# ownzonefeng/pytorch-distributed-training-example

Hardware: AMD Instinct MI355X
Metric: images/sec (whole node) ResNet-50 DDP at 1/2/4/8 MI355X; scaling efficiency (higher is better)
Workload: dtype bf16; 1 GPU; model=resnet50, global_batch=1024, per_gpu_batch=1024, image_size=224, parallelism=dp1, grad_accum=1, impl=ours, graph=False, precision=bf16, bucket_cap_mb=auto, comm_hook=none, reducer_active=True, pg_size=1, pg_backend=nccl, deterministic=False, full=False

## Files before the change

### pytorch_distributed_training_example_amd/config.py

```python
from __future__ import annotations

import os


class _Switches:
    __slots__ = ("disable_native", "conv1x1", "conv1x1_ours", "conv1x1_prefer", "conv1x1_override",
                 "conv1x1_table", "conv1x1_dump", "conv1x1_s2", "conv3x3", "conv3x3_wgrad", "conv3x3_s2", "conv_stem",
                 "conv_bn_stats", "bn_bwd_stats", "res_masked", "stem_bwd_fused", "stem_bn_wgrad", "stem_bn_stats", "stem_pool_wgrad", "wgrad_splitk", "slice_sum",
                 "subsample_native", "linear_splitk", "fused_addln", "embedding_native", "linear_epilogue",
                 "bwd_fused", "bwd_fused_shapes", "bwd_alg", "alg_glo", "bwd_alg_min_m", "z3_virtual", "bwd_alg_first", "ds_alg", "bn2_defer", "bn_apply_gemm_k", "strided_bstats", "gap_native", "sub_out",
                 "fp8_fused_gelu", "fp8_weight_multi", "fp8_cast_colsum", "fp8_ln", "wgrad_stream_m",
                 "dropout_fused")

    def __init__(self):
        self.reload()

    def reload(self) -> "_Switches":
        e = os.environ.get

        def on(name: str, default: str = "1") -> bool:
            return e(name, default) != "0"

        self.disable_native = e("PDT_DISABLE_NATIVE", "0") == "1"
        self.conv1x1 = e("PDT_CONV1X1", "auto")
# ... 2 lines not shown
        ov = e("PDT_CONV1X1_OVERRIDE", "")
        self.conv1x1_override = dict(p.split("=", 1) for p in ov.replace("+", ";").split(";") if "=" in p)
        self.conv1x1_table = on("PDT_CONV1X1_TABLE")
        self.conv1x1_dump = e("PDT_CONV1X1_DUMP") or None
        self.conv1x1_s2 = e("PDT_CONV1X1_S2", "1") == "1"
        self.conv3x3 = e("PDT_CONV3X3", "ours")
        self.conv3x3_wgrad = e("PDT_CONV3X3_WGRAD", "ours")
        self.conv3x3_s2 = e("PDT_CONV3X3_S2", "ours")
        self.conv_stem = e("PDT_CONV_STEM", "ours")
        self.conv_bn_stats = on("PDT_CONV_BN_STATS")
        self.bn_bwd_stats = on("PDT_BN_BWD_STATS")
        self.res_masked = on("PDT_RES_MASKED")
        self.stem_bwd_fused = on("PDT_STEM_BWD_FUSED")
        self.stem_bn_wgrad = on("PDT_STEM_BN_WGRAD")
        self.stem_bn_stats = on("PDT_STEM_BN_STATS")
        self.stem_pool_wgrad = on("PDT_STEM_POOL_WGRAD")
        self.wgrad_splitk = on("PDT_WGRAD_SPLITK")
        self.slice_sum = on("PDT_SLICE_SUM")
        self.subsample_native = on("PDT_SUBSAMPLE_NATIVE")
        self.linear_splitk = on("PDT_LINEAR_SPLITK")
        self.fused_addln = on("PDT_FUSED_ADDLN")
        self.embedding_native = on("PDT_EMBEDDING_NATIVE")
        self.linear_epilogue = e("PDT_LINEAR_EPILOGUE", "auto")
        self.bwd_fused = on("PDT_BWD_FUSED")
        self.bwd_fused_shapes = tuple(tuple(int(v) for v in t.split("x")) for t in
                                      e("PDT_BWD_FUSED_SHAPES", "256x64").split(",") if "x" in t)
        self.bwd_alg = int(e("PDT_BWD_ALG", "2"))
        self.bwd_alg_min_m = int(e("PDT_BWD_ALG_MIN_M", "50176"))
        self.alg_glo = on("PDT_ALG_GLO", "1")
        self.z3_virtual = int(e("PDT_Z3_VIRTUAL", "2"))
        self.bwd_alg_first = on("PDT_BWD_ALG_FIRST", "1")
        self.ds_alg = int(e("PDT_DS_ALG", "512"))
        self.bn2_defer = on("PDT_BN2_DEFER", "0")
        self.bn_apply_gemm_k = int(e("PDT_BN_APPLY_GEMM_K", "128"))
        self.strided_bstats = on("PDT_STRIDED_BSTATS")
        self.gap_native = on("PDT_GAP_NATIVE")
        self.sub_out = on("PDT_SUB_OUT")
        self.fp8_fused_gelu = on("PDT_FP8_FUSED_GELU")
        self.fp8_weight_multi = on("PDT_FP8_WEIGHT_MULTI")
        self.fp8_cast_colsum = on("PDT_FP8_CAST_COLSUM")
        self.fp8_ln = on("PDT_FP8_LN")
        self.wgrad_stream_m = int(e("PDT_WGRAD_STREAM_M", "0"))
        self.dropout_fused = on("PDT_DROPOUT_FUSED")
        return self


SW = _Switches()
```

### pytorch_distributed_training_example_amd/csrc/binding.cpp

```cpp
#include <torch/extension.h>
#include <ATen/hip/HIPContext.h>

#include <cstring>
#include <map>
#include <vector>

#include "fp8_pack.h"
#include "launchers.h"

namespace {

using at::Tensor;

hipStream_t stream() { return at::hip::getCurrentHIPStream().stream(); }

int dcode(const Tensor& t) {
  if (t.scalar_type() == at::kFloat) return 0;
  if (t.scalar_type() == at::kBFloat16) return 1;
  TORCH_CHECK(false, "pdt: unsupported dtype ", t.scalar_type(), " (fp32 / bf16 only)");
}

void check_cuda(const Tensor& t, const char* name) {
  TORCH_CHECK(t.is_cuda(), "pdt: ", name, " must be a GPU tensor");
}
// ... 2306 lines not shown
  m.doc() = "gfx950 HIP kernels for pytorch_distributed_training_example_amd";
  m.def("sgd", &sgd);
  m.def("adam", &adam);
  m.def("adadelta", &adadelta);
  m.def("lars", &lars);
  m.def("lamb", &lamb);
  m.def("layerwise_chunks", &layerwise_chunks);
  m.def("amp_unscale", &amp_unscale);
  m.def("amp_update", &amp_update);
  m.def("mt_scale", &mt_scale);
  m.def("mt_copy", &mt_copy);
  m.def("l2norm_sq", &l2norm_sq);
  m.def("clip_coef", &clip_coef);
  m.def("bn_tune", [](int variant, int target_blocks, int u_fwd, int u_bwd) {
    if (pdt_bn_tune(variant, target_blocks, u_fwd, u_bwd) != 0)
      throw py::value_error("bn_tune: variant must be 0 (keep), 3 (in-kernel finalize) or 5 (finalize kernel), got " +
                            std::to_string(variant));
  }, py::arg("variant") = 0, py::arg("target_blocks") = 0, py::arg("u_fwd") = 0, py::arg("u_bwd") = 0);
  m.def("bn_fwd_train", &bn_fwd_train, py::arg("x"), py::arg("res"), py::arg("weight"), py::arg("bias"),
        py::arg("running_mean"), py::arg("running_var"), py::arg("momentum"), py::arg("eps"), py::arg("relu"),
        py::arg("res_ab") = py::none(), py::arg("apply") = true);
  m.def("bn_fwd_eval", &bn_fwd_eval);
  m.def("bn_relu_maxpool_fwd", &bn_relu_maxpool_fwd);
  m.def("bn_relu_maxpool_fwd_parts", &bn_relu_maxpool_fwd_parts);
  m.def("maxpool3s2_bwd", &maxpool3s2_bwd);
  m.def("conv1x1_gemm", &conv1x1_gemm, py::arg("a"), py::arg("b"), py::arg("out"), py::arg("acc"), py::arg("stats"),
        py::arg("c_in") = py::none(), py::arg("c_mask") = py::none(), py::arg("bn_x") = py::none(),
        py::arg("bn_mask") = py::none(), py::arg("bn_mean") = py::none(), py::arg("c_stride") = 0,
        py::arg("c_H") = 0, py::arg("c_W") = 0, py::arg("a_coef") = py::none(), py::arg("bn_sum_only") = false,
        py::arg("no_store") = false);
  m.def("conv1x1_probe", [](int probe) { pdt_conv1x1_probe(probe); });
  m.def("conv1x1_persist", [](int mode) { return pdt_conv1x1_persist(mode); },
        "1x1 GEMM persistence mode (0 off, 1 measured kinds, 2 all, -1 env default); returns the previous mode");
  m.def("conv1x1_last_persistent", []() { return pdt_conv1x1_last_persistent(); },
        "which kernel the last 1x1 GEMM call launched: 0 one tile per workgroup, else the persistent kernel's waves "
        "per workgroup (+256 statistics-only, +512 APPLY)");
  m.def("conv3x3_opt", [](int v) { return pdt_conv3x3_opt(v); },
        "3x3 conv variant bits (csrc/kernels/conv3x3.hip conv3x3_opt; -1 env default); returns the previous value");
  m.def("weight_prep", &weight_prep);
  m.def("bn_tiles_fused", [](int on) { pdt_bn_tiles_fused(on); });
  m.def("maxpool_bwd_v2", [](int on) { pdt_maxpool_bwd_v2(on); });
  m.def("pool_fwd_contig", [](int on) { pdt_pool_fwd_contig(on); });
  m.def("bn_apply_wgs", [](int n) { pdt_bn_apply_wgs(n); });
  m.def("bn_row_wgs", [](int n) { pdt_bn_row_wgs(n); });
  m.def("gap_bwd", &gap_bwd, py::arg("g"), py::arg("H"), py::arg("W"), py::arg("bn_x") = py::none(),
        py::arg("bn_mask") = py::none(), py::arg("bn_mean") = py::none(), py::arg("bn_sum_only") = false);
  m.def("conv1x1_gemm_apply", &conv1x1_gemm_apply, py::arg("a"), py::arg("b"), py::arg("res"), py::arg("ab"),
        py::arg("rab") = py::none(), py::arg("a_coef") = py::none());
  m.def("bn_bwd_train_tiles", &bn_bwd_train_tiles);
  m.def("maxpool3s2_bwd_bn", &maxpool3s2_bwd_bn);
  m.def("maxpool3s2_bwd_bn_coef", &maxpool3s2_bwd_bn_coef, py::arg("dy"), py::arg("code"), py::arg("x"),
        py::arg("weight"), py::arg("mean"), py::arg("invstd"), py::arg("need_dgamma"), py::arg("write_dz") = true);
  m.def("slice_sum", &slice_sum);
  m.def("subsample_gather", &subsample_gather);
  m.def("subsample_scatter_add", &subsample_scatter_add);
  m.def("bn_fwd_train_tiles", &bn_fwd_train_tiles, py::arg("x"), py::arg("part"), py::arg("res"), py::arg("weight"),
        py::arg("bias"), py::arg("running_mean"), py::arg("running_var"), py::arg("momentum"), py::arg("eps"),
        py::arg("relu"), py::arg("res_ab") = py::none(), py::arg("apply") = true, py::arg("sub") = 0);
  m.def("conv3x3s1_variant", &conv3x3s1_variant);
  m.def("conv3x3_wgrad_geo", &conv3x3_wgrad_geo);
  m.def("conv3x3s1_fwd", &conv3x3s1_fwd);
  m.def("conv3x3s1_fwd_stats", &conv3x3s1_fwd_stats);
  m.def("conv3x3s1_fwd_bnbwd", &conv3x3s1_fwd_bnbwd);
  m.def("conv3x3_flip", &conv3x3_flip);
  m.def("conv3x3s2_fwd", &conv3x3s2_fwd);
  m.def("conv3x3s2_wgrad", &conv3x3s2_wgrad);
// ... 95 lines not shown
```

### pytorch_distributed_training_example_amd/csrc/kernels/conv1x1.hip

```cpp
#include "../common.h"
#include "../launchers.h"
#include "../tile_stats.h"

#include <stdlib.h>

using namespace pdt;

namespace {

typedef __bf16 bf16x8 __attribute__((ext_vector_type(8)));
typedef float f4 __attribute__((ext_vector_type(4)));
#define PDT_LDS __attribute__((address_space(3)))

__device__ __attribute__((aligned(256))) uint4 g_gemm_zero[16];
__device__ __attribute__((aligned(256))) uint4 g_gemm_ones[16] = {
    {0x3f803f80u, 0x3f803f80u, 0x3f803f80u, 0x3f803f80u}, {0x3f803f80u, 0x3f803f80u, 0x3f803f80u, 0x3f803f80u},
    {0x3f803f80u, 0x3f803f80u, 0x3f803f80u, 0x3f803f80u}, {0x3f803f80u, 0x3f803f80u, 0x3f803f80u, 0x3f803f80u},
    {0x3f803f80u, 0x3f803f80u, 0x3f803f80u, 0x3f803f80u}, {0x3f803f80u, 0x3f803f80u, 0x3f803f80u, 0x3f803f80u},
    {0x3f803f80u, 0x3f803f80u, 0x3f803f80u, 0x3f803f80u}, {0x3f803f80u, 0x3f803f80u, 0x3f803f80u, 0x3f803f80u},
    {0x3f803f80u, 0x3f803f80u, 0x3f803f80u, 0x3f803f80u}, {0x3f803f80u, 0x3f803f80u, 0x3f803f80u, 0x3f803f80u},
    {0x3f803f80u, 0x3f803f80u, 0x3f803f80u, 0x3f803f80u}, {0x3f803f80u, 0x3f803f80u, 0x3f803f80u, 0x3f803f80u},
    {0x3f803f80u, 0x3f803f80u, 0x3f803f80u, 0x3f803f80u}, {0x3f803f80u, 0x3f803f80u, 0x3f803f80u, 0x3f803f80u},
    {0x3f803f80u, 0x3f803f80u, 0x3f803f80u, 0x3f803f80u}, {0x3f803f80u, 0x3f803f80u, 0x3f803f80u, 0x3f803f80u}};
__device__ uint8_t g_mask_ones[16] = {
   0xff, 0xff, 0xff, 0xff, 0xff, 0xff, 0xff, 0xff,
                                            0xff, 0xff, 0xff, 0xff, 0xff, 0xff, 0xff, 0xff};

template <int BN_, int WM_, int WN_>
struct G1 {
  static constexpr int BM = 256, BN = BN_, WM = WM_, WN = WN_, BK = 32, kSlots = 3;
  static constexpr int kWaves = WM * WN, kThreads = kWaves * 64;
  static constexpr int kABytes = BM * 64, kBBytes = BN * 64, kSlot = kABytes + kBBytes;
  static constexpr int kEpiStride = BN * 2 + 16;
  static constexpr int kEpi = BM * kEpiStride;
  static constexpr int kRed = 0;
  static constexpr int kLds = kSlots * kSlot > kEpi + kRed ? kSlots * kSlot : kEpi + kRed;
  static constexpr int kMB = BM / WM / 16, kNB = BN / WN / 16;
  static constexpr int kALd = BM / 16 / kWaves, kBLd = BN / 16 / kWaves, kG = kALd + kBLd;
  static constexpr int kOcc = (160 * 1024) / kLds;
  static constexpr int kMinWaves = kOcc * kThreads / 256 > 0 ? kOcc * kThreads / 256 : 1;
  static_assert(kALd * 16 * kWaves == BM && kBLd * 16 * kWaves == BN, "DMA split");
};

__device__ __forceinline__ int chk64(int row, int p) { return p ^ (((row >> 2) & 1) << 1); }
__device__ __forceinline__ int swz64(int row, int chunk) { return row * 64 + (chk64(row, chunk) << 4); }

__device__ __forceinline__ f4 mfma(bf16x8 a, bf16x8 b, f4 c) {
  return __builtin_amdgcn_mfma_f32_16x16x32_bf16(a, b, c, 0, 0, 0);
}

__device__ __forceinline__ void dma16(const void* src, char* lds_wave_base) {
  __builtin_amdgcn_global_load_lds(src, (PDT_LDS void*)lds_wave_base, 16, 0, 0);
}

template <int G>
__device__ __forceinline__ void wait_vm() {
  static_assert(G >= 0 && G <= 6, "vmcnt");
  if constexpr (G == 6) asm volatile("s_waitcnt vmcnt(6)" ::: "memory");
  else if constexpr (G == 5) asm volatile("s_waitcnt vmcnt(5)" ::: "memory");
  else if constexpr (G == 4) asm volatile("s_waitcnt vmcnt(4)" ::: "memory");
  else if constexpr (G == 3) asm volatile("s_waitcnt vmcnt(3)" ::: "memory");
  else if constexpr (G == 2) asm volatile("s_waitcnt vmcnt(2)" ::: "memory");
  else if constexpr (G == 1) asm volatile("s_waitcnt vmcnt(1)" ::: "memory");
  else asm volatile("s_waitcnt vmcnt(0)" ::: "memory");
}

typedef unsigned u32x4 __attribute__((ext_vector_type(4)));

struct CGeom {
  int s, H, W, Hs, Ws;
};

struct ApArgs {
  const float* ab;
// ... 289 lines not shown
                                   mt, N, n0);
  }
}

template <class Cf, int HV = 0>
struct PL {
  static constexpr int kStgOff = 2 * Cf::kSlot;
  static constexpr int kFull = Cf::BM * Cf::kEpiStride;
  static constexpr int kHalves = HV > 0 ? HV : (kStgOff + kFull <= 152 * 1024 ? 1 : 2);
  static_assert(Cf::WM % kHalves == 0, "a part is whole wave rows");
  static constexpr int kStg = kFull / kHalves;
  static constexpr int kRed0 = Cf::kWaves * (Cf::BN / 8) * 16 * 4, kRed1 = Cf::kWaves * 2 * Cf::BN * 4;
  static constexpr int kRed = kRed0 > kRed1 ? kRed0 : kRed1;
  static constexpr int kArea = kStg > kRed ? kStg : kRed;
  static constexpr int kLds = 3 * Cf::kSlot > kStgOff + kArea ? 3 * Cf::kSlot : kStgOff + kArea;
  static constexpr int kOcc = (160 * 1024) / kLds;
  static constexpr int kMinWaves = kOcc * Cf::kThreads / 256 > 0 ? kOcc * Cf::kThreads / 256 : 1;
  static_assert(kLds <= 160 * 1024 && kFull % kHalves == 0, "LDS");
};

__device__ __attribute__((aligned(256))) uint4 g_gemm_sink[1024];
__device__ uint8_t g_mask_sink[1024];

__device__ __forceinline__ void dma16a(const void* src, char* lds_wave_base) {
  const uint32_t m0 = __builtin_amdgcn_readfirstlane((uint32_t)(uintptr_t)(PDT_LDS const char*)lds_wave_base);
  asm volatile("s_mov_b32 m0, %1\n\ts_nop 0\n\tglobal_load_lds_dwordx4 %0, off" ::"v"(src), "s"(m0) : "memory");
}
template <int N>
__device__ __forceinline__ void wait_vmn() {
  static_assert(N >= 0 && N < 64, "vmcnt");
  __builtin_amdgcn_s_waitcnt((N & 15) | (7 << 4) | (15 << 8) | ((N >> 4) << 14));
}

template <class Cf, bool ACC, bool STATS, bool BSTATS, bool ATR, bool APPLY, bool STR, bool NOST = false, int HV = 0>
__global__ __launch_bounds__(Cf::kThreads, (PL<Cf, HV>::kMinWaves)) void conv1x1p_kernel(
    const uint16_t* __restrict__ A, const uint16_t* __restrict__ B, uint16_t* Y, const uint16_t* Cin,
    const uint8_t* __restrict__ Cmask, float* __restrict__ part, int M, int K, int N, BnSrc bs, CGeom cg,
    const float* __restrict__ acoef, ApArgs ap) {
  static_assert(!(APPLY && (ACC || STATS || BSTATS)), "APPLY is a forward epilogue of its own");
  static_assert(!STR || ACC, "STR: a strided accumulate source");
  static_assert(!NOST || (STATS && !ACC && !BSTATS && !APPLY), "NOST: the statistics-only forward");
  using L = PL<Cf, HV>;
  constexpr int BM = Cf::BM, BN = Cf::BN, kG = Cf::kG, kHalves = L::kHalves;
  constexpr int WROWS = BM / Cf::WM, WCOLS = BN / Cf::WN;
  extern __shared__ __attribute__((aligned(16))) char lds[];
  const int tid = threadIdx.x, lane = tid & 63, wid = __builtin_amdgcn_readfirstlane(tid >> 6);
  const int wm = wid % Cf::WM, wn = wid / Cf::WM;
  const int ntn = N / BN, T = (M + BM - 1) / BM, total = T * ntn;
  const int G = gridDim.x, xg = blockIdx.x % 8, jg = blockIdx.x / 8, gx = (G - xg + 7) / 8;
  const int c_lo = (int)((int64_t)total * xg / 8), c_hi = (int)((int64_t)total * (xg + 1) / 8);
  int tile = c_lo + jg;
  if (tile >= c_hi) return;
  const int S = K / Cf::BK;
  char* const stg = lds + L::kStgOff;

  const int sub = lane >> 2, p = lane & 3;
  auto aoff_of = [&](int m0, int i) {
    const int r = (wid * Cf::kALd + i) * 16 + sub;
    return m0 + r < M ? (m0 + r) * K + chk64(r, p) * 8 : -1;
  };
  auto boff_of = [&](int n0, int j) {
    const int r = (wid * Cf::kBLd + j) * 16 + sub;
    return (n0 + r) * K + chk64(r, p) * 8;
  };
  int aoff[Cf::kALd], boff[Cf::kBLd];
  auto issue = [&](int s, int slot_i) {
    char* slot = lds + slot_i * Cf::kSlot;
    const int ko = s * Cf::BK;
#pragma unroll
    for (int i = 0; i < Cf::kALd; ++i)
      dma16a(aoff[i] >= 0 ? (const void*)(A + (aoff[i] + ko)) : (const void*)g_gemm_zero, slot + (wid * Cf::kALd + i) * 1024);
#pragma unroll
    for (int j = 0; j < Cf::kBLd; ++j) dma16a(B + (boff[j] + ko), slot + Cf::kABytes + (wid * Cf::kBLd + j) * 1024);
  };
// ... 19 lines not shown
  const uint16_t* const bx_base = bs.x ? bs.x : reinterpret_cast<const uint16_t*>(g_gemm_zero);
  const int64_t bx_scale = bs.x ? 1 : 0;

  int mt = tile / ntn, n0 = (tile % ntn) * BN, m0 = mt * BM;
  int tab_n0 = -1;
#pragma unroll
  for (int i = 0; i < Cf::kALd; ++i) aoff[i] = aoff_of(m0, i);
#pragma unroll
  for (int j = 0; j < Cf::kBLd; ++j) boff[j] = boff_of(n0, j);
  issue(0, 0);
  if (S > 1) issue(1, 1);
  bool first = true;
  const int lrow = lane & 15, lchk = lane >> 4;
  for (;;) {
    f4 acc[Cf::kMB][Cf::kNB];
#pragma unroll
    for (int i = 0; i < Cf::kMB; ++i)
#pragma unroll
      for (int j = 0; j < Cf::kNB; ++j) acc[i][j] = f4{0.f, 0.f, 0.f, 0.f};
    for (int s = 0; s < S; ++s) {
      const bool nxt = s + 1 < S;
      if (s >= 2 || first) {
        if (nxt) wait_vmn<kG>(); else wait_vmn<0>();
      } else {
        if (nxt) wait_vmn<kG + kStores>(); else wait_vmn<kStores>();
      }
      __builtin_amdgcn_s_barrier();
      asm volatile("" ::: "memory");
      if (s + 2 < S) issue(s + 2, (s + 2) % 3);
      const char* As = lds + (s % 3) * Cf::kSlot;
      const char* Bs = As + Cf::kABytes;
      bf16x8 a[Cf::kMB], b[Cf::kNB];
#pragma unroll
      for (int i = 0; i < Cf::kMB; ++i) a[i] = *reinterpret_cast<const bf16x8*>(As + swz64(wm * WROWS + i * 16 + lrow, lchk));
#pragma unroll
      for (int j = 0; j < Cf::kNB; ++j) b[j] = *reinterpret_cast<const bf16x8*>(Bs + swz64(wn * WCOLS + j * 16 + lrow, lchk));
      if constexpr (ATR) {
        const int k0 = s * Cf::BK + 8 * lchk;
        float ca[8], cb[8];
        *reinterpret_cast<float4*>(ca) = *reinterpret_cast<const float4*>(ctab + k0);
        *reinterpret_cast<float4*>(ca + 4) = *reinterpret_cast<const float4*>(ctab + k0 + 4);
        *reinterpret_cast<float4*>(cb) = *reinterpret_cast<const float4*>(ctab + K + k0);
        *reinterpret_cast<float4*>(cb + 4) = *reinterpret_cast<const float4*>(ctab + K + k0 + 4);
#pragma unroll
        for (int i = 0; i < Cf::kMB; ++i) {
          typedef unsigned u4 __attribute__((ext_vector_type(4)));
          const u4 w = __builtin_bit_cast(u4, a[i]);
          u4 o;
#pragma unroll
          for (int k = 0; k < 4; ++k) {
            const float t0 = __uint_as_float(w[k] << 16) * ca[2 * k] + cb[2 * k];
            const float t1 = __uint_as_float(w[k] & 0xffff0000u) * ca[2 * k + 1] + cb[2 * k + 1];
            o[k] = (uint32_t)f2bf(t0 > 0.f ? t0 : 0.f) | ((uint32_t)f2bf(t1 > 0.f ? t1 : 0.f) << 16);
          }
          a[i] = __builtin_bit_cast(bf16x8, o);
        }
      }
#pragma unroll
      for (int i = 0; i < Cf::kMB; ++i)
#pragma unroll
        for (int j = 0; j < Cf::kNB; ++j) acc[i][j] = mfma(b[j], a[i], acc[i][j]);
      asm volatile("s_waitcnt lgkmcnt(0)" ::: "memory");
    }

    uint2 pk[Cf::kMB][Cf::kNB];
#pragma unroll
    for (int i = 0; i < Cf::kMB; ++i)
// ... 9 lines not shown
    const int next = tile + gx;
    const bool has_next = next < c_hi;
    if (has_next) {
      mt = next / ntn; n0 = (next % ntn) * BN; m0 = mt * BM;
#pragma unroll
      for (int i = 0; i < Cf::kALd; ++i) aoff[i] = aoff_of(m0, i);
#pragma unroll
      for (int j = 0; j < Cf::kBLd; ++j) boff[j] = boff_of(n0, j);
      issue(0, 0);
      if (S > 1) issue(1, 1);
    }

    RowStats8 rst;
    float kst = 0.f;
    float bs1[8], bs2[8], bmu[8];
    if constexpr (APPLY) {
      if (cur_n0 != tab_n0) {
        if (tid < BN) {
          atab[tid] = ap.ab[cur_n0 + tid];
          atab[BN + tid] = ap.ab[N + cur_n0 + tid];
          atab[2 * BN + tid] = ap.rab ? ap.rab[cur_n0 + tid] : 1.f;
          atab[3 * BN + tid] = ap.rab ? ap.rab[N + cur_n0 + tid] : 0.f;
        }
        tab_n0 = cur_n0;
      }
    }
    if constexpr (BSTATS) {
      *reinterpret_cast<float4*>(bmu) = *reinterpret_cast<const float4*>(bs.mean + cur_n0 + c * 8);
      *reinterpret_cast<float4*>(bmu + 4) = *reinterpret_cast<const float4*>(bs.mean + cur_n0 + c * 8 + 4);
#pragma unroll
      for (int k = 0; k < 8; ++k) { bs1[k] = 0.f; bs2[k] = 0.f; }
    }
#pragma unroll
    for (int hv = 0; hv < kHalves; ++hv) {
      constexpr int kWH = Cf::WM / kHalves;
      if (wm / kWH == hv) {
#pragma unroll
        for (int i = 0; i < Cf::kMB; ++i)
#pragma unroll
          for (int j = 0; j < Cf::kNB; ++j) {
            const int ml = (wm % kWH) * WROWS + i * 16 + lrow;
            const int cl = wn * WCOLS + j * 16 + 4 * lchk;
            *reinterpret_cast<uint2*>(stg + ml * Cf::kEpiStride + cl * 2) = pk[i][j];
          }
      }
      asm volatile("s_waitcnt lgkmcnt(0)" ::: "memory");
      __builtin_amdgcn_s_barrier();
      asm volatile("" ::: "memory");
      if constexpr (STATS) {
        if (hv == 0) {
          rs8_init(rst, *reinterpret_cast<const uint4*>(stg + (tid % kChunks) * 16));
          if (tid < BN) kst = __uint_as_float((uint32_t)*reinterpret_cast<const uint16_t*>(stg + tid * 2) << 16);
        }
      }
#pragma unroll
      for (int h = hv * kItH; h < (hv + 1) * kItH; h += kB) {
        uint4 cv[kB], xbv[kB];
        unsigned cmk[kB], bmkv[kB];
        bool okv[kB];
#pragma unroll
        for (int it = 0; it < kB; ++it) {
          const int m = cur_m0 + r0 + kRowStep * (h + it);
          const bool ok = m < M;
          okv[it] = ok;
          const int mc = ok ? m : M - 1;
          const int64_t off = (int64_t)mc * N + cur_n0 + c * 8;
          if constexpr (BSTATS) {
// ... 57 lines not shown
                const float rf = __uint_as_float(k & 1 ? wr & 0xffff0000u : wr << 16);
                float t = zf * fa[k] + fb[k];
                t += ap.rab ? rf * fra[k] + frb[k] : rf;
                amb |= (t > 0.f ? 1u : 0u) << (4 * q + k);
                z[k] = t > 0.f ? t : 0.f;
              }
              o[2 * q] = (uint32_t)f2bf(z[0]) | ((uint32_t)f2bf(z[1]) << 16);
              o[2 * q + 1] = (uint32_t)f2bf(z[2]) | ((uint32_t)f2bf(z[3]) << 16);
            }
            v = make_uint4(o[0], o[1], o[2], o[3]);
          }
          if constexpr (BSTATS) {
            bn_bwd_accum8(v, xbv[it], bmkv[it], bmu, bs1, bs2);
            v = mask8(v, bmkv[it]);
          }
          if constexpr (STATS) {
            if (ok) rs8_add(rst, v);
          }
          if constexpr (!NOST) {
            uint4* yp = ok ? reinterpret_cast<uint4*>(Y + off) : g_gemm_sink + tid;
            *yp = v;
          }
          if constexpr (APPLY) {
            uint8_t* mp = ok ? ap.mask + (off >> 3) : g_mask_sink + tid;
            *mp = (uint8_t)amb;
          }
        }
      }
      __builtin_amdgcn_s_barrier();
      asm volatile("" ::: "memory");
    }
    if constexpr (BSTATS)
      bn_bwd_tile_store<BN, Cf::kWaves>(bs1, bs2, reinterpret_cast<float*>(stg), bs.part, T, cur_mt, N, cur_n0);
    if constexpr (STATS)
      rs8_tile_store<BN, Cf::kWaves>(rst, kst, reinterpret_cast<float*>(stg), part, min(BM, M - cur_m0), T, cur_mt, N,
                                     cur_n0);
    if constexpr (BSTATS || STATS) {
      asm volatile("s_waitcnt lgkmcnt(0)" ::: "memory");
      __builtin_amdgcn_s_barrier();
      asm volatile("" ::: "memory");
    }
    if (!has_next) break;
    tile = next;
    first = false;
  }
  wait_vmn<0>();
}

int g_persist = -1;

inline int persist_mode() {
  if (g_persist < 0) {
    const char* e = getenv("PDT_CONV1X1_PERSIST");
    g_persist = (e && e[0]) ? (int)strtol(e, nullptr, 10) : 1;
    if (g_persist < 0 || g_persist > 2) g_persist = 1;
  }
  return g_persist;
}

int g_last_persistent = 0;

template <class Cf, bool ACC, bool STATS, bool BSTATS, bool ATR, bool APPLY, bool STR, bool NOST = false, int HV = 0>
int launch_p(const uint16_t* a, const uint16_t* b, uint16_t* y, const uint16_t* c, const uint8_t* cm, float* part, int M,
             int K, int N, const BnSrc& bs, const CGeom& cg, hipStream_t s, const float* acoef, const ApArgs& ap) {
  using L = PL<Cf, HV>;
  static bool attr = false;
  constexpr int kTab = APPLY ? 4 * Cf::BN * 4 : 0;
  constexpr int kMaxLds = L::kLds + (ATR ? 2 * 512 * 4 : 0) + kTab;
  static_assert(kMaxLds <= 160 * 1024, "LDS");
  if (!attr) {
    if (hipFuncSetAttribute(
            reinterpret_cast<const void*>(&conv1x1p_kernel<Cf, ACC, STATS, BSTATS, ATR, APPLY, STR, NOST, HV>),
            hipFuncAttributeMaxDynamicSharedMemorySize, kMaxLds) != hipSuccess)
      return -3;
    attr = true;
  }
  const int lds = L::kLds + (ATR ? 2 * K * 4 : 0) + kTab;
  const int64_t total = (int64_t)(M + Cf::BM - 1) / Cf::BM * (N / Cf::BN);
  const int occ = (160 * 1024) / lds > 0 ? (160 * 1024) / lds : 1;
  int64_t grid = 256 * (int64_t)occ;
  if (grid > total) grid = total;
  hipLaunchKernelGGL((conv1x1p_kernel<Cf, ACC, STATS, BSTATS, ATR, APPLY, STR, NOST, HV>), dim3((unsigned)grid),
                     dim3(Cf::kThreads), lds, s, a, b, y, c, cm, part, M, K, N, bs, cg, acoef, ap);
  g_last_persistent = Cf::kWaves | (NOST ? 256 : 0) | (APPLY ? 512 : 0);
  return 0;
}

constexpr int kMaxATRK = 512;

template <class Cf, bool ACC, bool STATS, bool NT, bool BSTATS, bool ATR = false, bool APPLY = false, bool STR = false,
          bool NOST = false>
int launch_nt(const uint16_t* a, const uint16_t* b, uint16_t* y, const uint16_t* c, const uint8_t* cm, float* part,
              int M, int K, int N, const BnSrc& bs, const CGeom& cg, hipStream_t s, const float* acoef = nullptr,
              const ApArgs& ap = ApArgs{}) {
  static bool attr = false;
  constexpr int kMaxLds = Cf::kLds + (ATR ? 2 * kMaxATRK * 4 : 0);
  if (!attr) {
    if (hipFuncSetAttribute(
            reinterpret_cast<const void*>(&conv1x1_kernel<Cf, ACC, STATS, NT, BSTATS, ATR, APPLY, STR, NOST>),
            hipFuncAttributeMaxDynamicSharedMemorySize, kMaxLds) != hipSuccess)
      return -3;
    attr = true;
  }
  if (ATR && K > kMaxATRK) return -1;
  const int lds = Cf::kLds + (ATR ? 2 * K * 4 : 0);
  const int64_t grid = (int64_t)(M + Cf::BM - 1) / Cf::BM * (N / Cf::BN);
  ApArgs apx = ap;
  apx.probe = g_probe;
  if constexpr (!NT) {
    constexpr int kHV = (APPLY && !ATR && Cf::kWaves == 8 && Cf::WM == 4) ? 4 : 0;
    constexpr bool kMeasured = (Cf::kWaves >= 16 && !ACC && !ATR && !APPLY) || (APPLY && !ATR && kHV == 4);
    const int pm = persist_mode();
    if ((pm == 2 || (pm == 1 && kMeasured)) && g_probe == 0 && !ap.a2 &&
        grid >= 2 * 256 * (int64_t)((160 * 1024) / PL<Cf, kHV>::kLds))
      return launch_p<Cf, ACC, STATS, BSTATS, ATR, APPLY, STR, NOST, kHV>(a, b, y, c, cm, part, M, K, N, bs, cg, s, acoef,
                                                                          apx);
  }
  hipLaunchKernelGGL((conv1x1_kernel<Cf, ACC, STATS, NT, BSTATS, ATR, APPLY, STR, NOST>), dim3((unsigned)grid),
                     dim3(Cf::kThreads), lds, s, a, b, y, c, cm, part, M, K, N, bs, cg, acoef, apx);
  g_last_persistent = 0;
  return 0;
}

template <class Cf, bool ACC, bool STATS, bool BSTATS = false>
int launch(const uint16_t* a, const uint16_t* b, uint16_t* y, const uint16_t* c, const uint8_t* cm, float* part, int M,
           int K, int N, const BnSrc& bs, const CGeom& cg, hipStream_t s, const ApArgs& ap = ApArgs{}) {
  if constexpr (ACC)
    if (cg.s) return launch_nt<Cf, ACC, STATS, false, BSTATS, false, false, true>(a, b, y, c, cm, part, M, K, N, bs, cg, s,
                                                                                  nullptr, ap);
  if constexpr (STATS && !ACC && !BSTATS)
    if (ap.nostore)
      return launch_nt<Cf, false, true, false, false, false, false, false, true>(a, b, y, c, cm, part, M, K, N, bs, cg, s,
                                                                                 nullptr, ap);
  return launch_nt<Cf, ACC, STATS, false, BSTATS>(a, b, y, c, cm, part, M, K, N, bs, cg, s, nullptr, ap);
}

using GXWide = G1<256, 4, 4>;
using GWide = G1<128, 4, 2>;
using GNarrow = G1<64, 4, 1>;
using GXWide2 = G1<256, 2, 4>;
inline bool w2_on() {
  static const int v = [] {
    const char* e = getenv("PDT_CONV1X1_W2");
    return (e && e[0]) ? (int)strtol(e, nullptr, 10) : 0;
  }();
  return v != 0;
}

template <class Cf>
int dispatch(const uint16_t* a, const uint16_t* b, uint16_t* y, const uint16_t* c, const uint8_t* cm, float* part,
             int M, int K, int N, const BnSrc& bs, const CGeom& cg, hipStream_t s, const float* acoef = nullptr,
             const ApArgs& ap = ApArgs{}) {
  if ((c && part) || (cm && !c) || (part && bs.part) || (cg.s && (!c || cm))) return -1;
  if (acoef) {
    if (c || bs.part) return -1;
    if (part) return launch_nt<Cf, false, true, false, false, true>(a, b, y, c, cm, part, M, K, N, bs, cg, s, acoef);
    return launch_nt<Cf, false, false, false, false, true>(a, b, y, c, cm, part, M, K, N, bs, cg, s, acoef);
  }
  if (bs.part) {
    if (!bs.mean) return -1;
    if (c) return launch<Cf, true, false, true>(a, b, y, c, cm, part, M, K, N, bs, cg, s);
    return launch<Cf, false, false, true>(a, b, y, c, cm, part, M, K, N, bs, cg, s);
  }
  if (c) return launch<Cf, true, false>(a, b, y, c, cm, part, M, K, N, bs, cg, s);
  if (part) return launch<Cf, false, true>(a, b, y, c, cm, part, M, K, N, bs, cg, s, ap);
  return launch<Cf, false, false>(a, b, y, c, cm, part, M, K, N, bs, cg, s);
}

}

extern "C" {

int pdt_conv1x1_tile_rows() { return 256; }

void pdt_conv1x1_probe(int probe) { g_probe = probe; }

int pdt_conv1x1_persist(int mode) {
  const int old = persist_mode();
  g_persist = mode < 0 ? -1 : (mode > 2 ? 2 : mode);
  return old;
}

int pdt_conv1x1_last_persistent() { return g_last_persistent; }

int pdt_conv1x1_gemm(const uint16_t* a, const uint16_t* b, uint16_t* y, const uint16_t* c, const uint8_t* cm,
                     float* part, int M, int K, int N, const uint16_t* bn_x, const uint8_t* bn_mask,
                     const float* bn_mean, float* bn_part, int c_s, int c_H, int c_W, const float* acoef,
                     hipStream_t s, int nostore) {
  ApArgs ap{};
  ap.nostore = nostore && part && !c && !acoef && !bn_part ? 1 : 0;
  if (nostore && !ap.nostore) return -1;
  if (M < 1 || K < 32 || K % 32 != 0 || N < 64 || N % 64 != 0) return -1;
  if ((int64_t)M * (K > N ? K : N) >= ((int64_t)1 << 31) || (int64_t)N * K >= ((int64_t)1 << 31)) return -2;
  const BnSrc bs{bn_x, bn_mask, bn_mean, bn_part};
  CGeom cg{0, 1, 1, 1, 1};
  if (c_s > 0) {
    if (c_H < 1 || c_W < 1 || M % (c_H * c_W) != 0) return -1;
    cg = CGeom{c_s, c_H, c_W, (c_H - 1) / c_s + 1, (c_W - 1) / c_s + 1};
  }
  if (w2_on() && N % 256 == 0 && K >= 256 && !c && !acoef && !bs.part && !(g_probe & 64))
    return dispatch<GXWide2>(a, b, y, c, cm, part, M, K, N, bs, cg, s, acoef, ap);
  if (N % 256 == 0 && (int64_t)((M + 255) / 256) * (N / 256) >= 2048 && !(g_probe & 64) && !c && !acoef)
    return dispatch<GXWide>(a, b, y, c, cm, part, M, K, N, bs, cg, s, acoef, ap);
  if (N % 128 == 0 && !(g_probe & 8) && !small_grid_narrow((int64_t)((M + 255) / 256) * (N / 128)))
    return dispatch<GWide>(a, b, y, c, cm, part, M, K, N, bs, cg, s, acoef, ap);
  return dispatch<GNarrow>(a, b, y, c, cm, part, M, K, N, bs, cg, s, acoef, ap);
}

int pdt_conv1x1_gemm_seg(const uint16_t* a1, int k1, const uint16_t* a2, int k2, int rep2, const uint16_t* b,
                         uint16_t* y, int M, int N, const uint16_t* bn_x, const uint8_t* bn_mask, const float* bn_mean,
                         float* bn_part, hipStream_t s) {
  const int K = k1 + rep2 * k2 + 32;
// ... 51 lines not shown
```

### pytorch_distributed_training_example_amd/csrc/launchers.h

```cpp
#pragma once
#include <hip/hip_runtime.h>
#include <stdint.h>

extern "C" {

int pdt_amp_unscale(int n, void* const* g, const int64_t* numel, int dtype, const float* inv_scale, float* found_inf,
                    hipStream_t s);
int pdt_amp_update(float* scale, int* growth_tracker, const float* found_inf, float growth, float backoff,
                   int interval, hipStream_t s);
int pdt_mt_scale(int n, void* const* x, const int64_t* numel, int dtype, const float* scale_ptr, float scale,
                 hipStream_t s);
int pdt_mt_copy(int n, void* const* src, void* const* dst, const int64_t* numel, int sdt, int ddt,
                const float* scale_ptr, float scale, hipStream_t s);
int pdt_l2norm_sq(int n, void* const* x, const int64_t* numel, int dtype, float* out, hipStream_t s);
int pdt_clip_coef(const float* sumsq, float max_norm, float* coef, float* norm, hipStream_t s);

int pdt_attn_fwd(const uint16_t* q, const int64_t* qs, const uint16_t* k, const int64_t* ks, const uint16_t* v,
                 const int64_t* vs, uint16_t* o, const int64_t* os, float* lse, int B, int H, int T, int Dh,
                 int causal, float scale, hipStream_t s);
int pdt_attn_bwd(const uint16_t* dout, const int64_t* dos, const uint16_t* q, const int64_t* qs, const uint16_t* k,
                 const int64_t* ks, const uint16_t* v, const int64_t* vs, const uint16_t* o, const int64_t* os,
                 const float* lse, float* delta, uint16_t* dq, uint16_t* dk, uint16_t* dv, const int64_t* gs, int B,
                 int H, int T, int Dh, int causal, float scale, hipStream_t s);
int pdt_attn_fwd_drop(const uint16_t* q, const int64_t* qs, const uint16_t* k, const int64_t* ks, const uint16_t* v,
// ... 61 lines not shown
int pdt_maxpool_bn_parts(int N, int H);
int pdt_maxpool3s2_bwd_bn(const uint16_t* dy, const uint8_t* code, uint16_t* dz, int N, int H, int W, int C,
                          const uint16_t* x, const float* gamma, const float* mean, const float* invstd, uint16_t* dx,
                          float* dgamma, float* dbeta, float* part, float* ws, hipStream_t s);
int pdt_maxpool3s2_bwd_bn_coef(const uint16_t* dy, const uint8_t* code, uint16_t* dz, int N, int H, int W, int C,
                               const uint16_t* x, const float* gamma, const float* mean, const float* invstd,
                               float* coef, float* dgamma, float* dbeta, float* part, float* ws, hipStream_t s);
int pdt_bn_sync_fwd_stats(const uint16_t* x, int64_t M, int C, float* stats, float* count, float* ws,
                          unsigned* counters, hipStream_t s);
int pdt_bn_sync_fwd_merge(const float* gathered, int W, int C, const float* gamma, const float* beta,
                          float* running_mean, float* running_var, float momentum, float eps, float* mean,
                          float* invstd, float* ab, int64_t* ntot, hipStream_t s);
int pdt_bn_apply_coef(const uint16_t* x, const uint16_t* res, const float* ab, int64_t M, int C, int relu,
                      uint16_t* y, uint8_t* mask, hipStream_t s);
int pdt_bn_sync_bwd_sums(const uint16_t* dy, const uint16_t* x, const uint8_t* mask, const float* mean, int64_t M,
                         int C, int relu, float* sums, float* ws, unsigned* counters, hipStream_t s);
int pdt_bn_sync_bwd_merge(const float* gathered, int W, int rank, int C, const float* gamma, const float* invstd,
                          const int64_t* ntot, float* coef, float* dgamma, float* dbeta, hipStream_t s);
int pdt_bn_bwd_apply_coef(const uint16_t* dy, const uint16_t* x, const uint8_t* mask, const float* mean,
                          const float* coef, int64_t M, int C, int relu, int has_res, uint16_t* dx, uint16_t* dres,
                          hipStream_t s);

int pdt_bn_alg_fix_s2(float* part, int T, const float* wg, const uint16_t* W, int C4, int CW, hipStream_t s);
int pdt_bn_alg_ds_part(float* part, const float* s1, const float* mean, const float* wg, const uint16_t* W, int C4,
                       int CW, hipStream_t s);
int pdt_bn_alg_small_gemm(const uint16_t* W, const uint16_t* Wt, const float* coef, const float* wg, float* G,
                          float* BWG, int C4, int CW, hipStream_t s);
int pdt_bn_alg_assemble(const uint16_t* W, const float* coef, const float* mean, const float* G, const float* wg,
                        const float* BWG, uint16_t* bcat, uint16_t* dW, int C4, int CW, int rep, hipStream_t s);

int pdt_conv1x1_tile_rows();
void pdt_conv1x1_probe(int probe);
int pdt_conv1x1_persist(int mode);
int pdt_conv1x1_last_persistent();
int pdt_conv1x1_gemm(const uint16_t* a, const uint16_t* b, uint16_t* y, const uint16_t* c, const uint8_t* cm,
                     float* part, int M, int K, int N, const uint16_t* bn_x, const uint8_t* bn_mask,
                     const float* bn_mean, float* bn_part, int c_s, int c_H, int c_W, const float* acoef,
                     hipStream_t s, int nostore);
int pdt_conv1x1_gemm_seg(const uint16_t* a1, int k1, const uint16_t* a2, int k2, int rep2, const uint16_t* b,
                         uint16_t* y, int M, int N, const uint16_t* bn_x, const uint8_t* bn_mask,
                         const float* bn_mean, float* bn_part, hipStream_t s);
int pdt_conv1x1_gemm_apply(const uint16_t* a, const uint16_t* b, uint16_t* y, const uint16_t* res, const float* ab,
                           const float* rab, uint8_t* mask, int M, int K, int N, const float* acoef, hipStream_t s);

int pdt_conv1x1_bwd_fused_ok(int C4, int CW);
int pdt_conv1x1_bwd_fused_grid(int M, int C4, int CW);
int pdt_conv1x1_bwd_fused(const uint16_t* dy, const uint16_t* z, const uint8_t* mz, const float* mean, const float* A,
                          const float* B, const float* D, const uint16_t* wt, const uint16_t* xa, const uint16_t* bx,
                          const uint8_t* bm, const float* bmean, float* bpart, const float* xcoef, uint8_t* mask_out,
                          uint16_t* dxa, uint16_t* dw, float* ws, int M, int C4, int CW, hipStream_t s);
void pdt_conv1x1_bwd_fused_tune(int grid);

int64_t pdt_conv1x1_wgrad_ws_floats(int M, int Ci, int Co, int* nsplit_out);
int pdt_conv1x1_wgrad(const uint16_t* x, const uint16_t* dy, uint16_t* dw, float* ws, int M, int Ci, int Co,
                      hipStream_t s);
int64_t pdt_conv1x1_wgrad_seg_ws_floats(int M, int Ci, int co1, int co2, int* rows_out);
int pdt_conv1x1_wgrad_seg(const uint16_t* x, const uint16_t* dy1, int co1, const uint16_t* dy2, int co2, float* out,
                          float* ws, int M, int Ci, hipStream_t s);
void pdt_conv1x1_wgrad_tune(int target_wgs, int variant, int interleave);

enum { PDT_C3_TAP_WIDE = 0, PDT_C3_TAP_NARROW, PDT_C3_HALO_WIDE, PDT_C3_HALO_NARROW, PDT_C3_WST, PDT_C3_WSR };
int pdt_conv3x3s1_variant(int N, int H, int W, int Ci, int Co);
int pdt_conv3x3s1_fwd(const uint16_t* x, const uint16_t* w, uint16_t* y, int N, int H, int W, int Ci, int Co,
                      hipStream_t s);
int pdt_conv3x3s1_stats_tile_rows(int N, int H, int W, int Ci, int Co);
int pdt_conv3x3s1_bnbwd_tile_rows(int N, int H, int W, int Ci, int Co);
// ... 176 lines not shown
```

### pytorch_distributed_training_example_amd/csrc/tile_stats.h

```cpp
#pragma once
#include <hip/hip_runtime.h>
#include <stdint.h>

namespace pdt {

template <int BM, int BN, int THREADS, int STRIDE>
__device__ __forceinline__ void tile_bn_stats(const char* tile, float* red, int nvalid, float* __restrict__ part,
                                              int mt, int T, int N, int n0) {
  constexpr int kGroups = THREADS / (BN / 2);
  constexpr int kRows = BM / kGroups;
  static_assert(BM % kGroups == 0, "row groups");
  const int tid = threadIdx.x;
  const int cp = tid % (BN / 2), g = tid / (BN / 2);
  const char* col = tile + cp * 4;
  float s0 = 0.f, s1 = 0.f;
#pragma unroll 8
  for (int rr = 0; rr < kRows; ++rr) {
    const int r = g * kRows + rr;
    const uint32_t v = *reinterpret_cast<const uint32_t*>(col + r * STRIDE);
    if (r < nvalid) { s0 += __uint_as_float(v << 16); s1 += __uint_as_float(v & 0xffff0000u); }
  }
  red[g * BN + 2 * cp] = s0;
  red[g * BN + 2 * cp + 1] = s1;
  __syncthreads();
// ... 12 lines not shown
    if (r < nvalid) { q0 += d0 * d0; q1 += d1 * d1; }
  }
  red[g * BN + 2 * cp] = q0;
  red[g * BN + 2 * cp + 1] = q1;
  __syncthreads();
  if (g == 0) {
    float m20 = 0.f, m21 = 0.f;
#pragma unroll
    for (int q = 0; q < kGroups; ++q) { m20 += red[q * BN + 2 * cp]; m21 += red[q * BN + 2 * cp + 1]; }
    *reinterpret_cast<float2*>(part + (int64_t)mt * N + n0 + 2 * cp) = make_float2(t0, t1);
    *reinterpret_cast<float2*>(part + ((int64_t)T + mt) * N + n0 + 2 * cp) = make_float2(m20, m21);
  }
}

template <int BM, int BN, int THREADS>
constexpr int tile_bn_stats_lds() { return (THREADS / (BN / 2)) * BN * 4; }

typedef float pdt_f2 __attribute__((ext_vector_type(2)));

struct RowStats8 {
  pdt_f2 k[4], s[4], q[4];
};

__device__ __forceinline__ void rs8_init(RowStats8& t, const uint4& k) {
  const uint32_t w[4] = {k.x, k.y, k.z, k.w};
#pragma unroll
  for (int j = 0; j < 4; ++j) {
    t.k[j] = pdt_f2{__uint_as_float(w[j] << 16), __uint_as_float(w[j] & 0xffff0000u)};
    t.s[j] = pdt_f2{0.f, 0.f};
    t.q[j] = pdt_f2{0.f, 0.f};
  }
}

__device__ __forceinline__ void rs8_add(RowStats8& t, const uint4& v) {
  const uint32_t w[4] = {v.x, v.y, v.z, v.w};
#pragma unroll
  for (int j = 0; j < 4; ++j) {
    const pdt_f2 d = pdt_f2{__uint_as_float(w[j] << 16), __uint_as_float(w[j] & 0xffff0000u)} - t.k[j];
    t.s[j] += d;
    t.q[j] = d * d + t.q[j];
  }
}

template <int BN, int WAVES>
__device__ __forceinline__ void rs8_tile_store(RowStats8& t, float K, float* red, float* __restrict__ part,
                                               int nvalid, int T, int mt, int N, int n0) {
  constexpr int kChunks = BN / 8;
  static_assert(64 % kChunks == 0, "chunk lanes");
  const int tid = threadIdx.x, lane = tid & 63, wid = tid >> 6;
  auto xr = [](float v) {
    if constexpr (kChunks <= 8) v = xor_add<8>(v);
    if constexpr (kChunks <= 16) v = xor_add<16>(v);
    return xor_add<32>(v);
  };
  static_assert(kChunks >= 8, "xor_add distances");
#pragma unroll
  for (int j = 0; j < 4; ++j) {
    t.s[j] = pdt_f2{xr(t.s[j].x), xr(t.s[j].y)};
    t.q[j] = pdt_f2{xr(t.q[j].x), xr(t.q[j].y)};
  }
  if (lane < kChunks) {
    float* r = red + (wid * kChunks + lane) * 16;
#pragma unroll
    for (int j = 0; j < 4; ++j) {
      r[2 * j] = t.s[j].x; r[2 * j + 1] = t.s[j].y;
      r[8 + 2 * j] = t.q[j].x; r[8 + 2 * j + 1] = t.q[j].y;
    }
  }
  __syncthreads();
  if (tid < BN) {
    const int c = tid >> 3, j = tid & 7;
    float S = 0.f, Q = 0.f;
#pragma unroll
    for (int w = 0; w < WAVES; ++w) {
      S += red[(w * kChunks + c) * 16 + j];
      Q += red[(w * kChunks + c) * 16 + 8 + j];
    }
    const float n = (float)nvalid;
    part[(int64_t)mt * N + n0 + tid] = fmaf(n, K, S);
    part[((int64_t)T + mt) * N + n0 + tid] = fmaxf(Q - S * S / n, 0.f);
  }
}

template <int BN, int WAVES>
constexpr int rs8_tile_store_lds() { return WAVES * (BN / 8) * 16 * 4; }

struct BnSrc {
  const uint16_t* x;
  const uint8_t* mask;
  const float* mean;
  float* part;
};

__device__ __forceinline__ void bn_bwd_accum8(uint4 v, uint4 xb, unsigned mk, const float (&mu)[8], float (&s1)[8],
                                              float (&s2)[8]) {
  const uint32_t w[4] = {v.x, v.y, v.z, v.w}, xw[4] = {xb.x, xb.y, xb.z, xb.w};
#pragma unroll
  for (int k = 0; k < 8; ++k) {
    const uint32_t gb = k & 1 ? (w[k >> 1] & 0xffff0000u) : (w[k >> 1] << 16);
    const uint32_t xv = k & 1 ? (xw[k >> 1] & 0xffff0000u) : (xw[k >> 1] << 16);
    const float g = (mk >> k) & 1u ? __uint_as_float(gb) : 0.f;
    s1[k] += g;
    s2[k] += g * (__uint_as_float(xv) - mu[k]);
  }
}

__device__ __forceinline__ uint4 mask8(uint4 v, unsigned mk) {
  uint32_t w[4] = {v.x, v.y, v.z, v.w};
#pragma unroll
  for (int k = 0; k < 4; ++k) {
    const uint32_t lo = (mk >> (2 * k)) & 1u ? 0x0000ffffu : 0u, hi = (mk >> (2 * k + 1)) & 1u ? 0xffff0000u : 0u;
    w[k] &= lo | hi;
  }
  return make_uint4(w[0], w[1], w[2], w[3]);
// ... 36 lines not shown
```

Before: 16600 images/sec.

## Compute 1x1 GEMM BN statistics directly from accumulator registers

```diff
diff --git a/pytorch_distributed_training_example_amd/config.py b/pytorch_distributed_training_example_amd/config.py
--- a/pytorch_distributed_training_example_amd/config.py
+++ b/pytorch_distributed_training_example_amd/config.py
@@ -58,7 +58,7 @@
         self.bwd_alg_first = on("PDT_BWD_ALG_FIRST", "1")
         self.ds_alg = int(e("PDT_DS_ALG", "512"))
         self.bn2_defer = on("PDT_BN2_DEFER", "0")
-        self.bn_apply_gemm_k = int(e("PDT_BN_APPLY_GEMM_K", "128"))
+        self.bn_apply_gemm_k = int(e("PDT_BN_APPLY_GEMM_K", "256"))
         self.strided_bstats = on("PDT_STRIDED_BSTATS")
         self.gap_native = on("PDT_GAP_NATIVE")
         self.sub_out = on("PDT_SUB_OUT")
diff --git a/pytorch_distributed_training_example_amd/csrc/binding.cpp b/pytorch_distributed_training_example_amd/csrc/binding.cpp
--- a/pytorch_distributed_training_example_amd/csrc/binding.cpp
+++ b/pytorch_distributed_training_example_amd/csrc/binding.cpp
@@ -2362,6 +2362,9 @@
   m.def("conv1x1_probe", [](int probe) { pdt_conv1x1_probe(probe); });
   m.def("conv1x1_persist", [](int mode) { return pdt_conv1x1_persist(mode); },
         "1x1 GEMM persistence mode (0 off, 1 measured kinds, 2 all, -1 env default); returns the previous mode");
+  m.def("conv1x1_nost_regs", [](int mode) { return pdt_conv1x1_nost_regs(mode); },
+        "statistics-only 16-wave persistent 1x1 GEMM: 1 statistics from the accumulator registers, 0 the staged "
+        "reduction, -1 env default; returns the previous mode");
   m.def("conv1x1_last_persistent", []() { return pdt_conv1x1_last_persistent(); },
         "which kernel the last 1x1 GEMM call launched: 0 one tile per workgroup, else the persistent kernel's waves "
         "per workgroup (+256 statistics-only, +512 APPLY)");
diff --git a/pytorch_distributed_training_example_amd/csrc/kernels/conv1x1.hip b/pytorch_distributed_training_example_amd/csrc/kernels/conv1x1.hip
--- a/pytorch_distributed_training_example_amd/csrc/kernels/conv1x1.hip
+++ b/pytorch_distributed_training_example_amd/csrc/kernels/conv1x1.hip
@@ -39,7 +39,12 @@
   static constexpr int kALd = BM / 16 / kWaves, kBLd = BN / 16 / kWaves, kG = kALd + kBLd;
   static constexpr int kOcc = (160 * 1024) / kLds;
   static constexpr int kMinWaves = kOcc * kThreads / 256 > 0 ? kOcc * kThreads / 256 : 1;
+  static constexpr bool kRegStats = false;
   static_assert(kALd * 16 * kWaves == BM && kBLd * 16 * kWaves == BN, "DMA split");
+};
+
+struct G1R : G1<256, 2, 8> {
+  static constexpr bool kRegStats = true;
 };
 
 __device__ __forceinline__ int chk64(int row, int p) { return p ^ (((row >> 2) & 1) << 1); }
@@ -395,6 +400,64 @@
   __builtin_amdgcn_s_waitcnt((N & 15) | (7 << 4) | (15 << 8) | ((N >> 4) << 14));
 }
 
+template <class Cf, class L>
+__device__ __forceinline__ void stats_from_regs(const f4 (&acc)[Cf::kMB][Cf::kNB], char* stg, float* __restrict__ part,
+                                                int nvalid, int T, int mt, int N, int n0, int wm, int wn, int lrow,
+                                                int lchk) {
+  constexpr int BN = Cf::BN, WCOLS = BN / Cf::WN;
+  static_assert(Cf::kMB == 8 && Cf::WM == 2 && WCOLS == 16 * Cf::kNB && BN / 8 == 32, "chains of 8 rows, 32 apart");
+  static_assert(L::kRed0 + BN * 4 <= L::kArea, "reduction area + shift line");
+  float* const red = reinterpret_cast<float*>(stg);
+  float* const kline = red + L::kRed0 / 4;
+  const int tid = threadIdx.x;
+  auto bf = [](float v) { return __uint_as_float((uint32_t)f2bf(v) << 16); };
+  if (wm == 0 && lrow == 0) {
+#pragma unroll
+    for (int j = 0; j < Cf::kNB; ++j) {
+      const f4 v = acc[0][j];
+      *reinterpret_cast<float4*>(kline + wn * WCOLS + j * 16 + 4 * lchk) = make_float4(bf(v[0]), bf(v[1]), bf(v[2]), bf(v[3]));
+    }
+  }
+  asm volatile("s_waitcnt lgkmcnt(0)" ::: "memory");
+  __builtin_amdgcn_s_barrier();
+  asm volatile("" ::: "memory");
+  const float kst = tid < BN ? kline[tid] : 0.f;
+  pdt_f2 ck[Cf::kNB][2], cs[Cf::kNB][2], cq[Cf::kNB][2];
+#pragma unroll
+  for (int j = 0; j < Cf::kNB; ++j) {
+    const float4 kv = *reinterpret_cast<const float4*>(kline + wn * WCOLS + j * 16 + 4 * lchk);
+    ck[j][0] = pdt_f2{kv.x, kv.y};
+    ck[j][1] = pdt_f2{kv.z, kv.w};
+    cs[j][0] = cs[j][1] = cq[j][0] = cq[j][1] = pdt_f2{0.f, 0.f};
+  }
+#pragma unroll
+  for (int t = 0; t < Cf::kMB; ++t) {
+    if ((2 * t + wm) * 16 + lrow < nvalid) {
+#pragma unroll
+      for (int j = 0; j < Cf::kNB; ++j) {
+        const f4 v = acc[t][j];
+        rs_pair_add(ck[j][0], cs[j][0], cq[j][0], pdt_f2{bf(v[0]), bf(v[1])});
+        rs_pair_add(ck[j][1], cs[j][1], cq[j][1], pdt_f2{bf(v[2]), bf(v[3])});
+      }
+    }
+  }
+  const int w = 8 * wm + (lrow >> 1);
+#pragma unroll
+  for (int j = 0; j < Cf::kNB; ++j) {
+    const float4 ps = make_float4(xor_add<1>(cs[j][0].x), xor_add<1>(cs[j][0].y), xor_add<1>(cs[j][1].x),
+                                  xor_add<1>(cs[j][1].y));
+    const float4 pq = make_float4(xor_add<1>(cq[j][0].x), xor_add<1>(cq[j][0].y), xor_add<1>(cq[j][1].x),
+                                  xor_add<1>(cq[j][1].y));
+    if (!(lrow & 1)) {
+      const int cl = wn * WCOLS + j * 16 + 4 * lchk;
+      float* r = red + (w * (BN / 8) + (cl >> 3)) * 16 + (cl & 7);
+      *reinterpret_cast<float4*>(r) = ps;
+      *reinterpret_cast<float4*>(r + 8) = pq;
+    }
+  }
+  rs8_tile_tail<BN, Cf::kWaves>(kst, red, part, nvalid, T, mt, N, n0);
+}
+
 template <class Cf, bool ACC, bool STATS, bool BSTATS, bool ATR, bool APPLY, bool STR, bool NOST = false, int HV = 0>
 __global__ __launch_bounds__(Cf::kThreads, (PL<Cf, HV>::kMinWaves)) void conv1x1p_kernel(
     const uint16_t* __restrict__ A, const uint16_t* __restrict__ B, uint16_t* Y, const uint16_t* Cin,
@@ -403,6 +466,8 @@
   static_assert(!(APPLY && (ACC || STATS || BSTATS)), "APPLY is a forward epilogue of its own");
   static_assert(!STR || ACC, "STR: a strided accumulate source");
   static_assert(!NOST || (STATS && !ACC && !BSTATS && !APPLY), "NOST: the statistics-only forward");
+  static_assert(!Cf::kRegStats || (NOST && !ATR && HV == 0), "G1R: the statistics-only tile");
+  constexpr bool REGS = Cf::kRegStats;
   using L = PL<Cf, HV>;
   constexpr int BM = Cf::BM, BN = Cf::BN, kG = Cf::kG, kHalves = L::kHalves;
   constexpr int WROWS = BM / Cf::WM, WCOLS = BN / Cf::WN;
@@ -488,7 +553,10 @@
       const char* Bs = As + Cf::kABytes;
       bf16x8 a[Cf::kMB], b[Cf::kNB];
 #pragma unroll
-      for (int i = 0; i < Cf::kMB; ++i) a[i] = *reinterpret_cast<const bf16x8*>(As + swz64(wm * WROWS + i * 16 + lrow, lchk));
+      for (int i = 0; i < Cf::kMB; ++i) {
+        const int ar = REGS ? (2 * i + wm) * 16 + lrow : wm * WROWS + i * 16 + lrow;
+        a[i] = *reinterpret_cast<const bf16x8*>(As + swz64(ar, lchk));
+      }
 #pragma unroll
       for (int j = 0; j < Cf::kNB; ++j) b[j] = *reinterpret_cast<const bf16x8*>(Bs + swz64(wn * WCOLS + j * 16 + lrow, lchk));
       if constexpr (ATR) {
@@ -564,7 +632,7 @@
       for (int k = 0; k < 8; ++k) { bs1[k] = 0.f; bs2[k] = 0.f; }
     }
 #pragma unroll
-    for (int hv = 0; hv < kHalves; ++hv) {
+    for (int hv = 0; hv < (REGS ? 0 : kHalves); ++hv) {
       constexpr int kWH = Cf::WM / kHalves;
       if (wm / kWH == hv) {
 #pragma unroll
@@ -688,9 +756,11 @@
     }
     if constexpr (BSTATS)
       bn_bwd_tile_store<BN, Cf::kWaves>(bs1, bs2, reinterpret_cast<float*>(stg), bs.part, T, cur_mt, N, cur_n0);
-    if constexpr (STATS)
+    if constexpr (STATS && !REGS)
       rs8_tile_store<BN, Cf::kWaves>(rst, kst, reinterpret_cast<float*>(stg), part, min(BM, M - cur_m0), T, cur_mt, N,
                                      cur_n0);
+    if constexpr (REGS)
+      stats_from_regs<Cf, L>(acc, stg, part, min(BM, M - cur_m0), T, cur_mt, N, cur_n0, wm, wn, lrow, lchk);
     if constexpr (BSTATS || STATS) {
       asm volatile("s_waitcnt lgkmcnt(0)" ::: "memory");
       __builtin_amdgcn_s_barrier();
@@ -712,6 +782,16 @@
     if (g_persist < 0 || g_persist > 2) g_persist = 1;
   }
   return g_persist;
+}
+
+int g_nost_regs = -1;
+
+inline int nost_regs_mode() {
+  if (g_nost_regs < 0) {
+    const char* e = getenv("PDT_CONV1X1_NOST_REGS");
+    g_nost_regs = (e && e[0]) ? (strtol(e, nullptr, 10) != 0 ? 1 : 0) : 1;
+  }
+  return g_nost_regs;
 }
 
 int g_last_persistent = 0;
@@ -768,9 +848,14 @@
     constexpr bool kMeasured = (Cf::kWaves >= 16 && !ACC && !ATR && !APPLY) || (APPLY && !ATR && kHV == 4);
     const int pm = persist_mode();
     if ((pm == 2 || (pm == 1 && kMeasured)) && g_probe == 0 && !ap.a2 &&
-        grid >= 2 * 256 * (int64_t)((160 * 1024) / PL<Cf, kHV>::kLds))
+        grid >= 2 * 256 * (int64_t)((160 * 1024) / PL<Cf, kHV>::kLds)) {
+      if constexpr (NOST && !ATR && Cf::BN == 256 && Cf::WM == 4 && Cf::WN == 4)
+        if (nost_regs_mode())
+          return launch_p<G1R, false, true, false, false, false, false, true>(a, b, y, c, cm, part, M, K, N, bs, cg, s,
+                                                                              acoef, apx);
       return launch_p<Cf, ACC, STATS, BSTATS, ATR, APPLY, STR, NOST, kHV>(a, b, y, c, cm, part, M, K, N, bs, cg, s, acoef,
                                                                           apx);
+    }
   }
   hipLaunchKernelGGL((conv1x1_kernel<Cf, ACC, STATS, NT, BSTATS, ATR, APPLY, STR, NOST>), dim3((unsigned)grid),
                      dim3(Cf::kThreads), lds, s, a, b, y, c, cm, part, M, K, N, bs, cg, acoef, apx);
@@ -834,6 +919,12 @@
 int pdt_conv1x1_persist(int mode) {
   const int old = persist_mode();
   g_persist = mode < 0 ? -1 : (mode > 2 ? 2 : mode);
+  return old;
+}
+
+int pdt_conv1x1_nost_regs(int mode) {
+  const int old = nost_regs_mode();
+  g_nost_regs = mode < 0 ? -1 : (mode ? 1 : 0);
   return old;
 }
 
diff --git a/pytorch_distributed_training_example_amd/csrc/launchers.h b/pytorch_distributed_training_example_amd/csrc/launchers.h
--- a/pytorch_distributed_training_example_amd/csrc/launchers.h
+++ b/pytorch_distributed_training_example_amd/csrc/launchers.h
@@ -117,6 +117,7 @@
 int pdt_conv1x1_tile_rows();
 void pdt_conv1x1_probe(int probe);
 int pdt_conv1x1_persist(int mode);
+int pdt_conv1x1_nost_regs(int mode);
 int pdt_conv1x1_last_persistent();
 int pdt_conv1x1_gemm(const uint16_t* a, const uint16_t* b, uint16_t* y, const uint16_t* c, const uint8_t* cm,
                      float* part, int M, int K, int N, const uint16_t* bn_x, const uint8_t* bn_mask,
diff --git a/pytorch_distributed_training_example_amd/csrc/tile_stats.h b/pytorch_distributed_training_example_amd/csrc/tile_stats.h
--- a/pytorch_distributed_training_example_amd/csrc/tile_stats.h
+++ b/pytorch_distributed_training_example_amd/csrc/tile_stats.h
@@ -68,13 +68,36 @@
   }
 }
 
+__device__ __forceinline__ void rs_pair_add(const pdt_f2& k, pdt_f2& s, pdt_f2& q, const pdt_f2& y) {
+  const pdt_f2 d = y - k;
+  s += d;
+  q = d * d + q;
+}
+
 __device__ __forceinline__ void rs8_add(RowStats8& t, const uint4& v) {
   const uint32_t w[4] = {v.x, v.y, v.z, v.w};
 #pragma unroll
-  for (int j = 0; j < 4; ++j) {
-    const pdt_f2 d = pdt_f2{__uint_as_float(w[j] << 16), __uint_as_float(w[j] & 0xffff0000u)} - t.k[j];
-    t.s[j] += d;
-    t.q[j] = d * d + t.q[j];
+  for (int j = 0; j < 4; ++j)
+    rs_pair_add(t.k[j], t.s[j], t.q[j], pdt_f2{__uint_as_float(w[j] << 16), __uint_as_float(w[j] & 0xffff0000u)});
+}
+
+template <int BN, int WAVES>
+__device__ __forceinline__ void rs8_tile_tail(float K, const float* red, float* __restrict__ part, int nvalid, int T,
+                                              int mt, int N, int n0) {
+  constexpr int kChunks = BN / 8;
+  const int tid = threadIdx.x;
+  __syncthreads();
+  if (tid < BN) {
+    const int c = tid >> 3, j = tid & 7;
+    float S = 0.f, Q = 0.f;
+#pragma unroll
+    for (int w = 0; w < WAVES; ++w) {
+      S += red[(w * kChunks + c) * 16 + j];
+      Q += red[(w * kChunks + c) * 16 + 8 + j];
+    }
+    const float n = (float)nvalid;
+    part[(int64_t)mt * N + n0 + tid] = fmaf(n, K, S);
+    part[((int64_t)T + mt) * N + n0 + tid] = fmaxf(Q - S * S / n, 0.f);
   }
 }
 
@@ -103,19 +126,7 @@
       r[8 + 2 * j] = t.q[j].x; r[8 + 2 * j + 1] = t.q[j].y;
     }
   }
-  __syncthreads();
-  if (tid < BN) {
-    const int c = tid >> 3, j = tid & 7;
-    float S = 0.f, Q = 0.f;
-#pragma unroll
-    for (int w = 0; w < WAVES; ++w) {
-      S += red[(w * kChunks + c) * 16 + j];
-      Q += red[(w * kChunks + c) * 16 + 8 + j];
-    }
-    const float n = (float)nvalid;
-    part[(int64_t)mt * N + n0 + tid] = fmaf(n, K, S);
-    part[((int64_t)T + mt) * N + n0 + tid] = fmaxf(Q - S * S / n, 0.f);
-  }
+  rs8_tile_tail<BN, WAVES>(K, red, part, nvalid, T, mt, N, n0);
 }
 
 template <int BN, int WAVES>
```

New measurement: 16740 images/sec, median of 6. No clear change (+0.9%).
